# CSB5/XNA_Basecaller

Measured on NVIDIA B200. Metric: signal samples/sec basecalled (sup@v3.3 XNA), higher is better.
Workload: dtype fp16

## Files before the change

### xna_basecaller_b200/csrc/conv3_gemm.cu

```cuda
#include "xb_common.cuh"
#include "xb_ptx.cuh"
#include "xb_gemm.cuh"

using namespace xbptx;

namespace {

constexpr int BM = 128, BN = 192, BK = 64;
constexpr int KBLK = XB_CONV3_K / BK;
constexpr int GROUPS = XB_FEATURES / BN;
constexpr int A_BYTES = BM * BK * 2, B_KB_BYTES = BN * BK * 2;
constexpr int STAGES = 4;
constexpr int STG_BYTES = 32 * 128;
constexpr int OFF_A = KBLK * B_KB_BYTES;
constexpr int OFF_STG = OFF_A + STAGES * A_BYTES;
constexpr int OFF_BIAS = OFF_STG + 8 * STG_BYTES;
constexpr int OFF_BAR = OFF_BIAS + BN * 4;
constexpr int SMEM_BYTES = OFF_BAR + 256 + 1024 ;
constexpr int THREADS = 384;
static_assert(XB_CONV3_K % BK == 0 && XB_FEATURES % BN == 0, "tile plan");
static_assert(OFF_A % 1024 == 0 && OFF_STG % 1024 == 0 && SMEM_BYTES <= 232448, "shared memory plan");

struct Conv3Params {
    int M, T, NB;
    const float *bias;
    const void *col;
    uint16_t *out;
};

__device__ __forceinline__ float tanh_approx(float x) {
    float y;
    asm("tanh.approx.f32 %0, %1;" : "=f"(y) : "f"(x));
    return y;
}
__device__ __forceinline__ void tma_store_3d(const CUtensorMap *m, uint32_t src_smem, int c0, int c1, int c2) {
    asm volatile("cp.async.bulk.tensor.3d.global.shared::cta.bulk_group [%0, {%2, %3, %4}], [%1];"
                 ::"l"(m), "r"(src_smem), "r"(c0), "r"(c1), "r"(c2) : "memory");
}
__device__ __forceinline__ void bulk_wait_group_read0() { asm volatile("cp.async.bulk.wait_group.read 0;" ::: "memory"); }

__global__ void __launch_bounds__(THREADS, 1)
conv3_kernel(const __grid_constant__ CUtensorMap tmA, const __grid_constant__ CUtensorMap tmB,
             const __grid_constant__ CUtensorMap tmO, const Conv3Params p) {
    extern __shared__ uint8_t smem_raw[];
    uint8_t *smem = reinterpret_cast<uint8_t *>((reinterpret_cast<uintptr_t>(smem_raw) + 1023) & ~uintptr_t(1023));
    float *sbias = reinterpret_cast<float *>(smem + OFF_BIAS);
    uint64_t *full = reinterpret_cast<uint64_t *>(smem + OFF_BAR);
    uint64_t *empty = full + STAGES;
    uint64_t *acc_full = empty + STAGES;
    uint64_t *acc_empty = acc_full + 2;
    uint64_t *w_full = acc_empty + 2;
    uint32_t *tmem_holder = reinterpret_cast<uint32_t *>(w_full + 1);

    const int warp = threadIdx.x >> 5, lane = threadIdx.x & 31;
    const int group = blockIdx.x % GROUPS, worker = blockIdx.x / GROUPS, workers = gridDim.x / GROUPS;
    const int n0 = group * BN;
    const int ntiles = (p.M + BM - 1) / BM;

    if (warp == 0 && lane == 0) {
        prefetch_tmap(&tmA);
        prefetch_tmap(&tmB);
        prefetch_tmap(&tmO);
        for (int s = 0; s < STAGES; s++) {
            mbar_init(&full[s], 1);
            mbar_init(&empty[s], 1);
        }
        for (int b = 0; b < 2; b++) {
            mbar_init(&acc_full[b], 1);
            mbar_init(&acc_empty[b], 4);
        }
        mbar_init(w_full, 1);
        fence_barrier_init();
    }
    if (warp == 2) {
        tmem_alloc(tmem_holder, 512);
        tmem_relinquish();
    }
    for (int i = threadIdx.x; i < BN; i += THREADS) sbias[i] = p.bias[n0 + i];
    tc_fence_before();
    __syncthreads();
    tc_fence_after();
    const uint32_t tmem_base = *tmem_holder;

    if (warp == 0) {
        if (elect_one()) {
            mbar_expect_tx(w_full, KBLK * B_KB_BYTES);
            for (int kb = 0; kb < KBLK; kb++) tma_load_2d(smem + kb * B_KB_BYTES, &tmB, w_full, kb * BK, n0);
            uint32_t it = 0;
            for (int tile = worker; tile < ntiles; tile += workers) {
                const int ahead = tile + 2 * workers;
                if (group == 0 && ahead < ntiles) {
                    const int rows = min(BM, p.M - ahead * BM);
                    const char *src = reinterpret_cast<const char *>(p.col) + (size_t)ahead * BM * (XB_CONV3_K * 2);
                    const uint32_t bytes = (uint32_t)rows * (XB_CONV3_K * 2);
                    for (uint32_t off = 0; off < bytes; off += 16384) prefetch_l2_bulk(src + off, min(16384u, bytes - off));
                }
                for (int kb = 0; kb < KBLK; kb++, it++) {
                    const int s = it % STAGES;
                    mbar_wait(&empty[s], ((it / STAGES) & 1) ^ 1);
                    mbar_expect_tx(&full[s], A_BYTES);
                    tma_load_2d(smem + OFF_A + s * A_BYTES, &tmA, &full[s], kb * BK, tile * BM);
                }
            }
        }
    } else if (warp == 1) {
        constexpr uint32_t idesc = umma_idesc_f16(0u, BM, BN);
        mbar_wait(w_full, 0);
        uint32_t it = 0, ti = 0;
        for (int tile = worker; tile < ntiles; tile += workers, ti++) {
            const int buf = ti & 1;
            mbar_wait(&acc_empty[buf], ((ti >> 1) & 1) ^ 1);
            tc_fence_after();
            const uint32_t d = tmem_base + buf * BN;
            for (int kb = 0; kb < KBLK; kb++, it++) {
                const int s = it % STAGES;
                mbar_wait(&full[s], (it / STAGES) & 1);
                tc_fence_after();
                if (elect_one()) {
                    const uint32_t a_addr = smem_u32(smem + OFF_A + s * A_BYTES);
                    const uint32_t b_addr = smem_u32(smem + kb * B_KB_BYTES);
#pragma unroll
                    for (int k = 0; k < BK / 16; k++)
                        mma_f16_ss(d, umma_desc_sw128(a_addr + k * 32), umma_desc_sw128(b_addr + k * 32), idesc, (kb | k) != 0);
                    mma_commit(&empty[s]);
                    if (kb == KBLK - 1) mma_commit(&acc_full[buf]);
                }
                __syncwarp();
            }
        }
    } else if (warp >= 4) {
        const int set = (warp - 4) >> 2, q = warp & 3;
        const uint32_t lane_base = tmem_base + ((uint32_t)(q * 32) << 16);
        const uint32_t stg = smem_u32(smem + OFF_STG + (set * 4 + q) * STG_BYTES);
        const uint32_t row_s = stg + lane * 128;
        uint32_t ti = 0;
        for (int tile = worker; tile < ntiles; tile += workers, ti++) {
            if ((int)(ti & 1) != set) continue;
            const int buf = ti & 1;
            mbar_wait(&acc_full[buf], (ti >> 1) & 1);
            tc_fence_after();
            const int m_w = tile * BM + q * 32;
            const int b_w = m_w / p.T, t_w = m_w - b_w * p.T;
#pragma unroll 1
            for (int cb = 0; cb < BN; cb += 64) {
                uint32_t a0[32], a1[32];
                tmem_ld_32x32b_x32(lane_base + buf * BN + cb, a0);
                tmem_ld_32x32b_x32(lane_base + buf * BN + cb + 32, a1);
                tmem_ld_wait();
                if (cb + 64 == BN) {
                    tc_fence_before();
                    __syncwarp();
                    if (lane == 0) mbar_arrive(&acc_empty[buf]);
                }
                const float *bs = sbias + cb;
                uint32_t pk[32];
#pragma unroll
                for (int e = 0; e < 32; e++) {
                    const int c = 2 * e;
                    float v0 = __uint_as_float(c < 32 ? a0[c & 31] : a1[c & 31]) + bs[c];
                    float v1 = __uint_as_float(c < 32 ? a0[(c + 1) & 31] : a1[(c + 1) & 31]) + bs[c + 1];
                    v0 = v0 * fmaf(tanh_approx(0.5f * v0), 0.5f, 0.5f);
                    v1 = v1 * fmaf(tanh_approx(0.5f * v1), 0.5f, 0.5f);
                    pk[e] = xb16<false>::pack(v0, v1);
                }
                if (lane == 0) bulk_wait_group_read0();
                __syncwarp();
#pragma unroll
                for (int j = 0; j < 8; j++)
                    sts_v4(row_s + (uint32_t)((j ^ (lane & 7)) << 4), make_uint4(pk[4 * j], pk[4 * j + 1], pk[4 * j + 2], pk[4 * j + 3]));
                if (t_w + 32 <= p.T) {
                    fence_proxy_async();
                    __syncwarp();
                    if (lane == 0) {
                        if (b_w < p.NB) tma_store_3d(&tmO, stg, n0 + cb, t_w, b_w);
                        bulk_commit_group();
                    }
                } else {
                    __syncwarp();
                    const int m = m_w + lane;
                    if (m < p.M) {
                        const int b = m / p.T, t = m - b * p.T;
                        uint16_t *o = p.out + ((size_t)t * p.NB + b) * XB_FEATURES + n0 + cb;
#pragma unroll
                        for (int j = 0; j < 8; j++)
                            reinterpret_cast<uint4 *>(o)[j] = lds_v4(row_s + (uint32_t)((j ^ (lane & 7)) << 4));
                    }
                    __syncwarp();
                }
            }
        }
        if (lane == 0) bulk_wait_group0();
        tc_fence_before();
    }
    __syncthreads();
    if (warp == 2) {
        tc_fence_after();
        tmem_dealloc(tmem_base, 512);
    }
}

}

int xb_conv3_launch(xb_handle *h, const void *col, const void *w3, const float *bias, void *out_tnc, int T, int N, cudaStream_t s) {
    const uint64_t M = (uint64_t)N * T;
    CUtensorMap tmA, tmB, tmO;
    if (int rc = xb_make_tmap_2d(h, &tmA, col, M, XB_CONV3_K, XB_CONV3_K)) return rc;
    if (int rc = xb_make_tmap_2d_box(h, &tmB, w3, XB_FEATURES, XB_CONV3_K, XB_CONV3_K, BK, BN, 1)) return rc;
    {
        const uint64_t dims[3] = {XB_FEATURES, (uint64_t)T, (uint64_t)N};
        const uint64_t st[2] = {(uint64_t)N * XB_FEATURES * 2, XB_FEATURES * 2};
        const uint32_t box[3] = {64, 32, 1};
        if (int rc = xb_make_tmap_nd(h, &tmO, out_tnc, 3, 2, dims, st, box)) return rc;
    }
    static bool configured[64] = {};
    if (!configured[h->device & 63]) {
        XB_CUDA(h, cudaFuncSetAttribute(conv3_kernel, cudaFuncAttributeMaxDynamicSharedMemorySize, SMEM_BYTES));
        configured[h->device & 63] = true;
    }
    Conv3Params p;
    p.M = (int)M; p.T = T; p.NB = N; p.bias = bias; p.col = col; p.out = reinterpret_cast<uint16_t *>(out_tnc);
    const int ntiles = (int)((M + BM - 1) / BM);
    int workers = (h->num_sms > 0 ? h->num_sms : 148) / GROUPS;
    if (workers > ntiles) workers = ntiles;
    conv3_kernel<<<GROUPS * workers, THREADS, SMEM_BYTES, s>>>(tmA, tmB, tmO, p);
    XB_LAUNCH_CHECK(h);
    return XB_OK;
}
```

### xna_basecaller_b200/csrc/conv_stem.cu

```cuda
#include "xb_common.cuh"

namespace {

constexpr int TT = 32;
constexpr int NP2 = 5 * TT + 14;
constexpr int NP1 = NP2 + 4;
constexpr int NPX = NP1 + 4;
constexpr int THREADS = 256;

__device__ __forceinline__ float swishf(float x) { return x * __fdividef(1.0f, 1.0f + __expf(-x)); }

template <typename SIG> __device__ __forceinline__ float load_sig(const SIG *p, size_t i);
template <> __device__ __forceinline__ float load_sig<float>(const float *p, size_t i) { return __ldg(p + i); }
template <> __device__ __forceinline__ float load_sig<__half>(const __half *p, size_t i) { return __half2float(p[i]); }
template <> __device__ __forceinline__ float load_sig<int16_t>(const int16_t *p, size_t i) { return (float)p[i]; }

template <bool BF16, typename SIG>
__global__ void __launch_bounds__(THREADS)
conv12_im2col_kernel(const SIG *__restrict__ signal, int L, int T, const float *__restrict__ w1,
                     const float *__restrict__ b1, const float *__restrict__ w2, const float *__restrict__ b2,
                     uint16_t *__restrict__ rows) {
    using X = xb16<BF16>;
    __shared__ float sx[NPX];
    __shared__ float s1[NP1][4];
    __shared__ __align__(16) uint16_t s2[NP2 + 1][16];
    __shared__ float sw1[20], sb1[4], sw2[320], sb2[16];

    const int b = blockIdx.y, t0 = blockIdx.x * TT, tid = threadIdx.x;
    const int p2_0 = 5 * t0 - 9;
    const int p1_0 = p2_0 - 2, px_0 = p1_0 - 2;
    const SIG *sig = signal + (size_t)b * L;

    for (int i = tid; i < 20; i += THREADS) sw1[i] = w1[i];
    for (int i = tid; i < 4; i += THREADS) sb1[i] = b1[i];
    for (int i = tid; i < 320; i += THREADS) sw2[i] = w2[i];
    for (int i = tid; i < 16; i += THREADS) sb2[i] = b2[i];
    for (int i = tid; i < NPX; i += THREADS) {
        int p = px_0 + i;
        sx[i] = (p >= 0 && p < L) ? load_sig<SIG>(sig, p) : 0.0f;
    }
    __syncthreads();
    for (int i = tid; i < NP1 * 4; i += THREADS) {
        int pos = i >> 2, ch = i & 3, p = p1_0 + pos;
        float v = 0.0f;
        if (p >= 0 && p < L) {
            v = sb1[ch];
#pragma unroll
            for (int k = 0; k < 5; k++) v = fmaf(sw1[ch * 5 + k], sx[pos + k], v);
            v = swishf(v);
        }
        s1[pos][ch] = v;
    }
    __syncthreads();
    for (int i = tid; i < (NP2 + 1) * 16; i += THREADS) {
        int pos = i >> 4, ch = i & 15, p = p2_0 + pos;
        float v = 0.0f;
        if (pos < NP2 && p >= 0 && p < L) {
            v = sb2[ch];
#pragma unroll
            for (int ci = 0; ci < 4; ci++)
#pragma unroll
                for (int k = 0; k < 5; k++) v = fmaf(sw2[(ch * 4 + ci) * 5 + k], s1[pos + k][ci], v);
            v = swishf(v);
        }
        typename X::T hv = X::from(v);
        s2[pos][ch] = *reinterpret_cast<uint16_t *>(&hv);
    }
    __syncthreads();
    const uint4 *s2v = reinterpret_cast<const uint4 *>(&s2[0][0]);
    for (int i = tid; i < TT * 40; i += THREADS) {
        int r = i / 40, v = i - r * 40, t = t0 + r;
        if (t >= T) continue;
        uint4 val = make_uint4(0, 0, 0, 0);
        if (v < 38) val = s2v[r * 10 + v];
        reinterpret_cast<uint4 *>(rows + ((size_t)b * T + t) * XB_CONV3_K)[v] = val;
    }
}

template <bool BF16, typename SIG>
int launch(xb_handle *h, const void *signal, int N, int L, cudaStream_t s) {
    const int T = L / XB_STRIDE;
    dim3 grid((T + TT - 1) / TT, N);
    conv12_im2col_kernel<BF16, SIG><<<grid, THREADS, 0, s>>>(reinterpret_cast<const SIG *>(signal), L, T, h->conv1_w,
                                                             h->conv1_b, h->conv2_w, h->conv2_b,
                                                             reinterpret_cast<uint16_t *>(h->c2));
    XB_LAUNCH_CHECK(h);
    return XB_OK;
}

}

int xb_conv12_im2col(xb_handle *h, const void *signal, int sig_dtype, int N, int L, cudaStream_t s) {
    switch (sig_dtype) {
        case XB_SIG_F32: return launch<false, float>(h, signal, N, L, s);
        case XB_SIG_F16: return launch<false, __half>(h, signal, N, L, s);
        case XB_SIG_I16: return launch<false, int16_t>(h, signal, N, L, s);
    }
    return xb_fail(h, XB_ERR_ARG, "unknown signal dtype %d", sig_dtype);
}
```

### xna_basecaller_b200/csrc/xb_api.cu

```cuda
#include <stdarg.h>
#include <stdlib.h>
#include <string.h>

#include "xb_common.cuh"
#include "xb_gemm.cuh"

thread_local std::string xb_global_err;

int xb_fail(xb_handle *h, int code, const char *fmt, ...) {
    char buf[512];
    va_list ap;
    va_start(ap, fmt);
    vsnprintf(buf, sizeof buf, fmt, ap);
    va_end(ap);
    if (h) h->err = buf;
    xb_global_err = buf;
    return code;
}

int xb_conv12_im2col(xb_handle *h, const void *signal, int sig_dtype, int N, int L, cudaStream_t s);
int xb_lstm_recurrence_persistent(xb_handle *h, int layer, void *y_tnc, int T, int N, int reverse, cudaStream_t s, void *save = nullptr);
int xb_inproj_launch(xb_handle *h, const void *x, const void *w_ih, const float *bias, void *gates, int M, cudaStream_t s);
int xb_head_astationary_launch(xb_handle *h, const void *x, const void *w, int w_rows, const float *bias, int head_rows,
                               float *scores, int ldo, int M, int exp_out, cudaStream_t s);
int xb_preprocess_impl(xb_handle *h, const int16_t *raw, const int64_t *read_offset, const int32_t *read_len,
                       const double *scaling, const int32_t *offset, int n_reads, float *out, int32_t *out_len,
                       float *stats, cudaStream_t s);
int xb_ctc_loss_bwd_impl(xb_handle *h, const float *scores, int T, int N, const int32_t *targets, int Lmax,
                         const int32_t *lengths, int normalise, const float *grad_loss, float *alpha_ws, float *grad,
                         cudaStream_t s);
int xb_ctc_loss_impl(xb_handle *h, const float *scores, int T, int N, const int32_t *targets, int Lmax,
                     const int32_t *lengths, int normalise, float *loss, cudaStream_t s);
int xb_stitch_impl(xb_handle *h, const int8_t *rows, int T, const int32_t *chunk_first, const int32_t *chunk_count,
                   const int32_t *read_len, int n_reads, int chunksize, int overlap, int stride, int reverse, int8_t *out,
                   int out_stride, int32_t *out_len, cudaStream_t s);

void xb_train_free(xb_handle *h);
int xb_beam_search_impl(xb_handle *h, const float *scores, const float *beta, int T, int N, int beam_width, float beam_cut,
                        int8_t *seq, int8_t *qstring, int8_t *moves, int32_t *lens, cudaStream_t s);
int xb_onehot_edges(xb_handle *h, const int32_t *edges_nt, int T, int N, int S, float *post, cudaStream_t s);
int xb_gather_chunks_impl(xb_handle *h, const void *signal, int sig_dtype, const int64_t *read_offset,
                          const int32_t *read_len, const int32_t *chunk_read, const int32_t *chunk_start, int n_chunks,
                          int L, float *out, cudaStream_t s);

namespace {

int ipow(int b, int e) { int r = 1; while (e-- > 0) r *= b; return r; }

template <typename T> int dev_alloc(xb_handle *h, T **p, size_t count) {
    void *q = nullptr;
    cudaError_t e = cudaMalloc(&q, count * sizeof(T));
    if (e != cudaSuccess)
        return xb_fail(h, XB_ERR_NOMEM, "cudaMalloc of %zu bytes failed: %s", count * sizeof(T), cudaGetErrorString(e));
    *p = reinterpret_cast<T *>(q);
    return XB_OK;
}
int dev_alloc_bytes(xb_handle *h, void **p, size_t bytes) { return dev_alloc<uint8_t>(h, reinterpret_cast<uint8_t **>(p), bytes); }

template <bool BF16>
__global__ void repack_kernel(const float *__restrict__ src, uint16_t *__restrict__ dst, int rows_dst, int cols_dst,
                              int rows_src, int cols_src, int mode) {
    size_t i = (size_t)blockIdx.x * blockDim.x + threadIdx.x;
    if (i >= (size_t)rows_dst * cols_dst) return;
    int r = (int)(i / cols_dst), c = (int)(i % cols_dst);
    float v = 0.0f;
    if (mode == 0) {
        if (r < rows_src && c < cols_src) v = src[(size_t)r * cols_src + c];
    } else if (mode == 1) {
        int j = r >> 7, g = (r >> 5) & 3, u = r & 31;
        v = src[(size_t)(g * XB_FEATURES + j * 32 + u) * cols_src + c];
    } else if (mode == 3) {
        int j = r >> 7, u = (r >> 2) & 31, g = r & 3;
        v = src[(size_t)(g * XB_FEATURES + j * 32 + u) * cols_src + c];
    } else if (mode == 4) {
        int j = r >> 7, q = (r >> 5) & 3, g = (r >> 3) & 3, ul = r & 7;
        v = src[(size_t)(g * XB_FEATURES + j * 32 + q * 8 + ul) * cols_src + c];
    } else if (mode == 5 || mode == 6) {
        if (mode == 5) { if (r < cols_src && c < rows_src) v = src[(size_t)c * cols_src + r]; }
        else {
            int tap = r >> 4, ch = r & 15;
            if (tap < XB_WINLEN) v = src[((size_t)c * XB_C2_CH + ch) * XB_WINLEN + tap];
        }
        __nv_bfloat16 bv = __float2bfloat16_rn(v);
        dst[i] = *reinterpret_cast<uint16_t *>(&bv);
        return;
    } else {
        int tap = c >> 4, ch = c & 15;
        if (tap < XB_WINLEN) v = src[((size_t)r * XB_C2_CH + ch) * XB_WINLEN + tap];
    }
    if (BF16) v = __bfloat162float(__float2bfloat16_rn(v));
    __half hv = __float2half_rn(v);
    dst[i] = *reinterpret_cast<uint16_t *>(&hv);
}
__global__ void lstm_bias_kernel(const float *__restrict__ b_ih, const float *__restrict__ b_hh, float *__restrict__ dst,
                                 int mode) {
    int r = blockIdx.x * blockDim.x + threadIdx.x;
    if (r >= XB_GATES) return;
    int j = r >> 7, g = (r >> 5) & 3, u = r & 31;
    if (mode == 3) { u = (r >> 2) & 31; g = r & 3; }
    int s = g * XB_FEATURES + j * 32 + u;
    dst[r] = b_ih[s] + b_hh[s];
}

// ... 14 lines not shown
    XB_REQUIRE(h, T > 0 && N > 0, "T and N must be positive (got T=%d N=%d)", T, N);
    XB_REQUIRE(h, T <= h->max_T && N <= h->max_N, "T=%d N=%d exceed the handle capacity max_T=%d max_N=%d", T, N, h->max_T,
               h->max_N);
    return XB_OK;
}

}

extern "C" {

int xb_abi_version(void) { return XB_ABI_VERSION; }

const char *xb_last_error(const xb_handle *h) { return h ? h->err.c_str() : xb_global_err.c_str(); }

int64_t xb_launch_count(const xb_handle *h) { return h ? h->launches : 0; }

int xb_set_profiling(xb_handle *h, int on) {
    if (!h) return xb_fail(nullptr, XB_ERR_ARG, "NULL handle");
    h->profiling = on != 0;
    return XB_OK;
}

int xb_stage_times(xb_handle *h, float *ms, int *spans) {
    if (!h) return xb_fail(nullptr, XB_ERR_ARG, "NULL handle");
    XB_REQUIRE(h, ms && spans, "NULL buffer");
    for (int i = 0; i < XB_ST_COUNT; i++) { ms[i] = 0.f; spans[i] = 0; }
    for (auto &sp : h->spans) {
        XB_CUDA(h, cudaEventSynchronize(sp.b));
        float t = 0.f;
        XB_CUDA(h, cudaEventElapsedTime(&t, sp.a, sp.b));
        ms[sp.stage] += t;
        spans[sp.stage]++;
        h->event_pool.push_back(sp.a);
        h->event_pool.push_back(sp.b);
    }
    h->spans.clear();
    return XB_OK;
}

int xb_create(xb_handle **out, int device, int max_N, int max_T, int n_base, int state_len, const char *alphabet, int flags) {
    if (!out) return xb_fail(nullptr, XB_ERR_ARG, "xb_create: out is NULL");
    *out = nullptr;
    if (max_N <= 0 || max_T <= 0) return xb_fail(nullptr, XB_ERR_ARG, "xb_create: max_N and max_T must be positive");
    if (!alphabet || (int)strlen(alphabet) != n_base + 1 || n_base + 1 > 15)
        return xb_fail(nullptr, XB_ERR_ARG, "xb_create: alphabet must have n_base+1 letters (blank first)");
    int key = n_base * 10 + state_len;
    if (!(key == 43 || key == 53 || key == 63 || key == 44 || key == 22))
        return xb_fail(nullptr, XB_ERR_UNSUPPORTED, "xb_create: no kernels for n_base=%d state_len=%d", n_base, state_len);
    int ndev = 0;
    cudaError_t e = cudaGetDeviceCount(&ndev);
    if (e != cudaSuccess || ndev == 0)
        return xb_fail(nullptr, XB_ERR_CUDA, "xb_create: no CUDA device (%s); this library has no CPU path",
                       cudaGetErrorString(e));
    if (device < 0 || device >= ndev) return xb_fail(nullptr, XB_ERR_ARG, "xb_create: device %d out of range", device);
    cudaDeviceProp prop;
    if (cudaGetDeviceProperties(&prop, device) != cudaSuccess || prop.major != 10)
        return xb_fail(nullptr, XB_ERR_UNSUPPORTED, "xb_create: device %d is not compute capability 10.x (sm_100a only)", device);
    if (cudaSetDevice(device) != cudaSuccess) return xb_fail(nullptr, XB_ERR_CUDA, "cudaSetDevice(%d) failed", device);

    xb_handle *h = new xb_handle();
    h->device = device;
    h->max_N = max_N;
    h->max_T = max_T;
    h->n_base = n_base;
    h->state_len = state_len;
    h->C = ipow(n_base, state_len);
    h->NZ = n_base + 1;
    h->flags = flags;
    h->bf16 = (flags & XB_FLAG_BF16) != 0;
    h->num_sms = prop.multiProcessorCount;
    strncpy(h->alphabet, alphabet, sizeof h->alphabet - 1);

    const size_t TN = (size_t)max_T * max_N, S = (size_t)h->C * h->NZ;
    int rc = XB_OK;
#define TRY(x) if (rc == XB_OK) rc = (x)
    const size_t VP = (size_t)((h->C + 31) / 32) * 32 + 4;
    TRY(dev_alloc(h, &h->alpha, (TN + max_N) * VP));
    TRY(dev_alloc(h, &h->bmax, (TN + max_N) * VP));
    TRY(dev_alloc(h, &h->lp, (TN + max_N) * VP));
    TRY(dev_alloc(h, &h->logz, (size_t)max_N));
    TRY(dev_alloc(h, &h->seq_dev, TN));
    TRY(dev_alloc(h, &h->lens_dev, (size_t)max_N));
    if (!(flags & XB_FLAG_NO_ENCODER)) {
        TRY(dev_alloc_bytes(h, &h->c2, TN * XB_CONV3_K * 2));
        TRY(dev_alloc_bytes(h, &h->act0, TN * XB_FEATURES * 2));
        TRY(dev_alloc_bytes(h, &h->act1, TN * XB_FEATURES * 2));
        TRY(dev_alloc_bytes(h, &h->gates, TN * XB_GATES * 2));
        TRY(dev_alloc(h, &h->cstate, (size_t)max_N * XB_FEATURES));
        TRY(dev_alloc(h, &h->scores, TN * S));
        TRY(dev_alloc_bytes(h, &h->signal_dev, TN * XB_STRIDE * sizeof(float)));
    }
#undef TRY
    if (rc != XB_OK) {
        xb_global_err = h->err;
        xb_destroy(h);
        return rc;
    }
    *out = h;
    return XB_OK;
}

int xb_destroy(xb_handle *h) {
    if (!h) return XB_OK;
    cudaSetDevice(h->device);
    void *ptrs[] = {h->conv1_w, h->conv1_b, h->conv2_w, h->conv2_b, h->conv3_w, h->conv3_b, h->head_w, h->head_b, h->c2,
                    h->act0, h->act1, h->gates, h->cstate, h->hzero, h->scores, h->signal_dev, h->seq_dev, h->lens_dev,
                    h->alpha, h->bmax, h->lp, h->logz, h->ctc_ws, h->lstm_counters};
    for (void *p : ptrs)
        if (p) cudaFree(p);
    for (void *p : {(void *)h->signal_dev2, (void *)h->seq_dev2, (void *)h->lens_dev2})
        if (p) cudaFree(p);
    if (h->h2d_stream) cudaStreamDestroy(h->h2d_stream);
    if (h->d2h_stream) cudaStreamDestroy(h->d2h_stream);
    for (int i = 0; i < 2; i++)
        for (cudaEvent_t e : {h->ev_h2d[i], h->ev_enc[i], h->ev_dec[i], h->ev_done[i]})
            if (e) cudaEventDestroy(e);
    for (auto &sp : h->spans) { cudaEventDestroy(sp.a); cudaEventDestroy(sp.b); }
    for (auto e : h->event_pool) cudaEventDestroy(e);
    for (auto &l : h->lstm) {
        for (void *p : {l.w_ih, l.w_hh, (void *)l.bias, l.w_ihT, l.w_hhT})
            if (p) cudaFree(p);
    }
    if (h->head_wT) cudaFree(h->head_wT);
    if (h->conv3_wT) cudaFree(h->conv3_wT);
    xb_train_free(h);
    delete h;
    return XB_OK;
}

static int alloc_weights(xb_handle *h) {
    if (h->conv1_w) return XB_OK;
    const int F = XB_FEATURES;
    h->head_rows = ipow(h->n_base, h->state_len + 1);
    h->head_rows_padded = ((h->head_rows + 127) / 128) * 128;
    int rc = XB_OK;
#define TRY(x) if (rc == XB_OK) rc = (x)
    TRY(dev_alloc(h, &h->conv1_w, 20));
    TRY(dev_alloc(h, &h->conv1_b, 4));
    TRY(dev_alloc(h, &h->conv2_w, 320));
    TRY(dev_alloc(h, &h->conv2_b, 16));
    TRY(dev_alloc_bytes(h, &h->conv3_w, (size_t)F * XB_CONV3_K * 2));
    TRY(dev_alloc(h, &h->conv3_b, (size_t)F));
    for (auto &l : h->lstm) {
        TRY(dev_alloc_bytes(h, &l.w_ih, (size_t)XB_GATES * F * 2));
        TRY(dev_alloc_bytes(h, &l.w_hh, (size_t)XB_GATES * F * 2));
        TRY(dev_alloc(h, &l.bias, (size_t)XB_GATES));
    }
    TRY(dev_alloc_bytes(h, &h->head_w, (size_t)h->head_rows_padded * F * 2));
    TRY(dev_alloc(h, &h->head_b, (size_t)h->head_rows_padded));
#undef TRY
    return rc;
}

#define XB_WEIGHTS_PROLOGUE()                                                                          \
    if (!h) return xb_fail(nullptr, XB_ERR_ARG, "NULL handle");                                        \
    XB_REQUIRE(h, !(h->flags & XB_FLAG_NO_ENCODER), "handle was created with XB_FLAG_NO_ENCODER");     \
    cudaStream_t s = reinterpret_cast<cudaStream_t>(stream);                                           \
    XB_CUDA(h, cudaSetDevice(h->device));                                                              \
    if (int rc_ = alloc_weights(h)) return rc_

int xb_load_conv_weights(xb_handle *h, const float *w1, const float *b1, const float *w2, const float *b2,
                         const float *w3, const float *b3, void *stream) {
    XB_WEIGHTS_PROLOGUE();
    XB_REQUIRE(h, w1 && b1 && w2 && b2 && w3 && b3, "NULL convolution weight");
    const int F = XB_FEATURES;
    XB_CUDA(h, cudaMemcpyAsync(h->conv1_w, w1, 20 * 4, cudaMemcpyDeviceToDevice, s));
    XB_CUDA(h, cudaMemcpyAsync(h->conv1_b, b1, 4 * 4, cudaMemcpyDeviceToDevice, s));
    XB_CUDA(h, cudaMemcpyAsync(h->conv2_w, w2, 320 * 4, cudaMemcpyDeviceToDevice, s));
    XB_CUDA(h, cudaMemcpyAsync(h->conv2_b, b2, 16 * 4, cudaMemcpyDeviceToDevice, s));
    if (int rc = repack(h, w3, h->conv3_w, F, XB_CONV3_K, F, XB_C2_CH * XB_WINLEN, 2, s)) return rc;
    if (h->flags & XB_FLAG_TRAIN) {
        if (!h->conv3_wT) { if (int rc = dev_alloc_bytes(h, &h->conv3_wT, (size_t)XB_CONV3_K * F * 2)) return rc; }
        if (int rc = repack(h, w3, h->conv3_wT, XB_CONV3_K, F, F, XB_C2_CH * XB_WINLEN, 6, s)) return rc;
    }
    XB_CUDA(h, cudaMemcpyAsync(h->conv3_b, b3, F * 4, cudaMemcpyDeviceToDevice, s));
    h->loaded |= 1;
    return XB_OK;
}

int xb_load_lstm_weights(xb_handle *h, int layer, const float *w_ih, const float *w_hh, const float *b_ih,
                         const float *b_hh, void *stream) {
    XB_WEIGHTS_PROLOGUE();
    XB_REQUIRE(h, layer >= 0 && layer < 5, "LSTM layer %d out of range", layer);
    XB_REQUIRE(h, w_ih && w_hh && b_ih && b_hh, "NULL LSTM weight");
    const int F = XB_FEATURES;
#ifdef XB_EXPERIMENTS
#define XB_FLAG_LSTM_STEPWISE 4
    const int ih_mode = (h->flags & XB_FLAG_LSTM_STEPWISE) ? 1 : 3;
#else
    const int ih_mode = 3;
#endif
    if (int rc = repack(h, w_ih, h->lstm[layer].w_ih, XB_GATES, F, XB_GATES, F, ih_mode, s)) return rc;
    if (int rc = repack(h, w_hh, h->lstm[layer].w_hh, XB_GATES, F, XB_GATES, F, ih_mode == 3 ? 4 : 1, s)) return rc;
    if (h->flags & XB_FLAG_TRAIN) {
        xb_lstm_weights &lw = h->lstm[layer];
        if (!lw.w_ihT) { if (int rc = dev_alloc_bytes(h, &lw.w_ihT, (size_t)XB_GATES * F * 2)) return rc; }
        if (!lw.w_hhT) { if (int rc = dev_alloc_bytes(h, &lw.w_hhT, (size_t)XB_GATES * F * 2)) return rc; }
        if (int rc = repack(h, w_ih, lw.w_ihT, F, XB_GATES, XB_GATES, F, 5, s)) return rc;
        if (int rc = repack(h, w_hh, lw.w_hhT, F, XB_GATES, XB_GATES, F, 5, s)) return rc;
    }
    lstm_bias_kernel<<<(XB_GATES + 255) / 256, 256, 0, s>>>(b_ih, b_hh, h->lstm[layer].bias, ih_mode);
    XB_LAUNCH_CHECK(h);
    h->loaded |= 2 << layer;
    return XB_OK;
}

int xb_load_head_weights(xb_handle *h, const float *w, const float *b, float scale, float blank_score,
                         int expand_blanks, void *stream) {
    XB_WEIGHTS_PROLOGUE();
    XB_REQUIRE(h, w != nullptr, "NULL head weight");
    const int F = XB_FEATURES;
    if (int rc = repack(h, w, h->head_w, h->head_rows_padded, F, h->head_rows, F, 0, s)) return rc;
    if (h->flags & XB_FLAG_TRAIN) {
        if (!h->head_wT) { if (int rc = dev_alloc_bytes(h, &h->head_wT, (size_t)h->head_rows_padded * F * 2)) return rc; }
        if (int rc = repack(h, w, h->head_wT, F, h->head_rows_padded, h->head_rows, F, 5, s)) return rc;
    }
    XB_CUDA(h, cudaMemsetAsync(h->head_b, 0, (size_t)h->head_rows_padded * 4, s));
    if (b) XB_CUDA(h, cudaMemcpyAsync(h->head_b, b, (size_t)h->head_rows * 4, cudaMemcpyDeviceToDevice, s));
    h->scale = scale;
    h->blank_score = blank_score;
    h->expand_blanks = expand_blanks;
    h->loaded |= 64;
    return XB_OK;
}

int xb_load_weights(xb_handle *h, const float *const *w, int n_tensors, float scale, float blank_score, int expand_blanks,
                    void *stream) {
    if (!h) return xb_fail(nullptr, XB_ERR_ARG, "xb_load_weights: NULL handle");
    XB_REQUIRE(h, w && n_tensors == XB_NUM_WEIGHTS, "expected %d weight tensors, got %d", XB_NUM_WEIGHTS, n_tensors);
    for (int i = 0; i < n_tensors; i++) XB_REQUIRE(h, w[i] != nullptr, "weight tensor %d is NULL", i);
    if (int rc = xb_load_conv_weights(h, w[0], w[1], w[2], w[3], w[4], w[5], stream)) return rc;
    for (int l = 0; l < 5; l++) {
        const float *const *lw = w + 6 + 4 * l;
        if (int rc = xb_load_lstm_weights(h, l, lw[0], lw[1], lw[2], lw[3], stream)) return rc;
    }
    return xb_load_head_weights(h, w[26], w[27], scale, blank_score, expand_blanks, stream);
}

int xb_conv_stem_fwd(xb_handle *h, const void *signal, int sig_dtype, int N, int L, void *out_tnc, void *stream) {
    if (!h) return xb_fail(nullptr, XB_ERR_ARG, "NULL handle");
    if (!(h->loaded & 1)) return xb_fail(h, XB_ERR_STATE, "convolution weights have not been loaded (xb_load_weights)");
    XB_REQUIRE(h, signal && out_tnc, "NULL buffer");
    XB_REQUIRE(h, L > 0 && L % XB_STRIDE == 0, "chunk length %d must be a positive multiple of the stride %d", L, XB_STRIDE);
    const int T = L / XB_STRIDE;
    if (int rc = check_tn(h, T, N)) return rc;
    cudaStream_t s = reinterpret_cast<cudaStream_t>(stream);
    {
        xb_stage_timer tm(h, XB_ST_CONV12, s);
        if (int rc = xb_conv12_im2col(h, signal, sig_dtype, N, L, s)) return rc;
    }
    xb_stage_timer tm(h, XB_ST_CONV3, s);
    return xb_conv3_launch(h, h->c2, h->conv3_w, h->conv3_b, out_tnc, T, N, s);
}

int xb_lstm_fwd(xb_handle *h, int layer, const void *x_tnc, void *y_tnc, int T, int N, int reverse, void *stream) {
    if (!h) return xb_fail(nullptr, XB_ERR_ARG, "NULL handle");
    XB_REQUIRE(h, layer >= 0 && layer < 5, "LSTM layer %d out of range", layer);
    if (!(h->loaded & (2 << layer))) return xb_fail(h, XB_ERR_STATE, "weights of LSTM layer %d have not been loaded", layer);
    XB_REQUIRE(h, x_tnc && y_tnc && x_tnc != y_tnc, "x and y must be distinct non-NULL buffers");
    if (int rc = check_tn(h, T, N)) return rc;
    cudaStream_t s = reinterpret_cast<cudaStream_t>(stream);
    const xb_lstm_weights &lw = h->lstm[layer];
    {
        xb_stage_timer tm(h, XB_ST_INPROJ, s);
#ifdef XB_EXPERIMENTS
        static const bool generic = getenv("XB_INPROJ_GENERIC") != nullptr;
        if (generic) {
            CUtensorMap tmA, tmB;
            if (int rc = xb_make_tmap_2d(h, &tmA, x_tnc, (uint64_t)T * N, XB_FEATURES, XB_FEATURES)) return rc;
            if (int rc = xb_make_tmap_2d(h, &tmB, lw.w_ih, XB_GATES, XB_FEATURES, XB_FEATURES)) return rc;
            GemmParams p;
            p.M = T * N; p.N = XB_GATES; p.K = XB_FEATURES;
            p.bias = lw.bias; p.out = h->gates; p.ldo = XB_GATES;
            if (int rc = xb_gemm_launch(h, EPI_INPROJ, tmA, tmB, p, s)) return rc;
        } else
#endif
        if (int rc = xb_inproj_launch(h, x_tnc, lw.w_ih, lw.bias, h->gates, T * N, s)) return rc;
    }
    xb_stage_timer tm(h, XB_ST_LSTM_REC, s);
#ifdef XB_EXPERIMENTS
    if (h->flags & XB_FLAG_LSTM_STEPWISE) {
        CUtensorMap tmH, tmW;
        if (int rc = xb_make_tmap_2d(h, &tmH, y_tnc, (uint64_t)T * N, XB_FEATURES, XB_FEATURES)) return rc;
        if (int rc = xb_make_tmap_2d(h, &tmW, lw.w_hh, XB_GATES, XB_FEATURES, XB_FEATURES)) return rc;
        for (int i = 0; i < T; i++) {
            const int t = reverse ? T - 1 - i : i;
            const int tp = reverse ? t + 1 : t - 1;
            GemmParams p;
            p.M = N; p.N = XB_GATES; p.K = XB_FEATURES;
            p.a_row_offset = (i == 0) ? 0 : tp * N;
            p.out = y_tnc; p.NB = N;
            p.gates = h->gates; p.cstate = h->cstate;
            p.t_cur = t; p.first = (i == 0);
            if (int rc = xb_gemm_launch(h, EPI_LSTM, tmH, tmW, p, s)) return rc;
        }
        return XB_OK;
    }
#endif
    return xb_lstm_recurrence_persistent(h, layer, y_tnc, T, N, reverse, s);
}

int xb_lstm_stack_fwd(xb_handle *h, void *x_tnc, void *y_tnc, int T, int N, void *stream) {
    if (!h) return xb_fail(nullptr, XB_ERR_ARG, "NULL handle");
    XB_REQUIRE(h, x_tnc && y_tnc && x_tnc != y_tnc, "x and y must be distinct non-NULL buffers");
    void *a = x_tnc, *b = y_tnc;
    for (int l = 0; l < 5; l++) {
        if (int rc = xb_lstm_fwd(h, l, a, b, T, N, (l % 2) == 0, stream)) return rc;
        void *t = a; a = b; b = t;
    }
    return XB_OK;
}

static int head_fwd(xb_handle *h, const void *x_tnc, float *scores, int T, int N, int exp_out, void *stream) {
    if (!h) return xb_fail(nullptr, XB_ERR_ARG, "NULL handle");
    if (!(h->loaded & 64)) return xb_fail(h, XB_ERR_STATE, "CRF head weights have not been loaded (xb_load_weights)");
    XB_REQUIRE(h, x_tnc && scores, "NULL buffer");
    if (int rc = check_tn(h, T, N)) return rc;
    cudaStream_t s = reinterpret_cast<cudaStream_t>(stream);
    xb_stage_timer tm(h, XB_ST_HEAD, s);
#ifdef XB_EXPERIMENTS
    static const bool tile_gemm = getenv("XB_HEAD_GENERIC") != nullptr;
    if (tile_gemm) {
        CUtensorMap tmA, tmB;
        if (int rc = xb_make_tmap_2d(h, &tmA, x_tnc, (uint64_t)T * N, XB_FEATURES, XB_FEATURES)) return rc;
        if (int rc = xb_make_tmap_2d(h, &tmB, h->head_w, h->head_rows_padded, XB_FEATURES, XB_FEATURES)) return rc;
        GemmParams p;
        p.M = T * N; p.N = h->head_rows_padded; p.K = XB_FEATURES;
        p.bias = h->head_b; p.out = scores;
        p.ldo = h->expand_blanks ? h->C * h->NZ : h->head_rows;
        p.n_base = h->n_base; p.head_rows = h->head_rows; p.expand = h->expand_blanks;
        p.scale = h->scale; p.blank = h->blank_score;
        return xb_gemm_launch(h, EPI_HEAD, tmA, tmB, p, s);
// ... 259 lines not shown
```

### xna_basecaller_b200/csrc/xb_common.cuh

```cuda
#pragma once

#include <cuda_runtime.h>
#include <cuda_fp16.h>
#include <cuda_bf16.h>
#include <cuda.h>
#include <stdint.h>
#include <stdio.h>
#include <string>
#include <vector>

#include "../../include/xna_basecaller.h"

#define XB_FEATURES 768
#define XB_GATES (4 * XB_FEATURES)
#define XB_STRIDE 5
#define XB_WINLEN 19
#define XB_C2_CH 16
#define XB_C2_HALO 9
#define XB_CONV3_K 320

struct xb_lstm_weights {
    void *w_ih = nullptr;
    void *w_hh = nullptr;
    float *bias = nullptr;
    void *w_ihT = nullptr;
    void *w_hhT = nullptr;
};

enum { XB_ST_CONV12 = 0, XB_ST_CONV3, XB_ST_INPROJ, XB_ST_LSTM_REC, XB_ST_HEAD, XB_ST_CRF_ALPHA, XB_ST_CRF_BACKWARD,
       XB_ST_CRF_VITERBI, XB_ST_TRAIN_BPTT, XB_ST_TRAIN_TRANSPOSE, XB_ST_TRAIN_WGRAD, XB_ST_TRAIN_XGRAD, XB_ST_TRAIN_HEAD_CONV,
       XB_ST_COUNT };

struct xb_prof_span { int stage; cudaEvent_t a, b; };

struct xb_handle {
    int device = 0;
    bool profiling = false;
    std::vector<xb_prof_span> spans;
    std::vector<cudaEvent_t> event_pool;
    int max_N = 0, max_T = 0;
    int n_base = 0, state_len = 0, C = 0, NZ = 0;
    int flags = 0;
    bool bf16 = false;
    int loaded = 0;
    char alphabet[16] = {0};
    int num_sms = 0;
    int64_t launches = 0;
    std::string err;

    float *conv1_w = nullptr, *conv1_b = nullptr, *conv2_w = nullptr, *conv2_b = nullptr;
    void *conv3_w = nullptr;
    float *conv3_b = nullptr;
    xb_lstm_weights lstm[5];
    void *head_w = nullptr;
    float *head_b = nullptr;
    int head_rows = 0, head_rows_padded = 0;
    float scale = 5.0f, blank_score = 2.0f;
    int expand_blanks = 1;

    void *c2 = nullptr;
    void *act0 = nullptr, *act1 = nullptr;
    void *gates = nullptr;
    float *cstate = nullptr;
    void *hzero = nullptr;
    float *scores = nullptr;
    void *signal_dev = nullptr;
    int8_t *seq_dev = nullptr;
    int32_t *lens_dev = nullptr;
    void *signal_dev2 = nullptr;
    int8_t *seq_dev2 = nullptr;
    int32_t *lens_dev2 = nullptr;
    cudaStream_t h2d_stream = nullptr, d2h_stream = nullptr;
    cudaEvent_t ev_h2d[2] = {nullptr, nullptr}, ev_enc[2] = {nullptr, nullptr}, ev_dec[2] = {nullptr, nullptr},
                ev_done[2] = {nullptr, nullptr};
    bool slot_used[2] = {false, false};

    float *alpha = nullptr;
    float *bmax = nullptr;
    float *lp = nullptr;
    float *logz = nullptr;
    float *ctc_ws = nullptr;
    int *lstm_counters = nullptr;

    void *head_wT = nullptr;
    void *conv3_wT = nullptr;
    struct xb_train_ws *train = nullptr;

    void *encode_tiled = nullptr;
};

extern thread_local std::string xb_global_err;

struct xb_stage_timer {
    xb_handle *h; cudaStream_t s; int idx = -1;
    xb_stage_timer(xb_handle *h_, int stage, cudaStream_t s_) : h(h_), s(s_) {
        if (!h->profiling) return;
        auto get = [&]() { cudaEvent_t e; if (!h->event_pool.empty()) { e = h->event_pool.back(); h->event_pool.pop_back(); }
                           else cudaEventCreate(&e); return e; };
        xb_prof_span sp{stage, get(), get()};
        cudaEventRecord(sp.a, s);
        h->spans.push_back(sp);
        idx = (int)h->spans.size() - 1;
// ... 64 lines not shown
```

### xna_basecaller_b200/csrc/xb_gemm.cuh

```cuda
#pragma once
#include "xb_common.cuh"

enum { EPI_F32 = 0, EPI_CONV3 = 1, EPI_INPROJ = 2, EPI_HEAD = 3, EPI_LSTM = 4, EPI_BF16OUT = 5, EPI_CONV3_BWD = 7 };

struct GemmParams {
    int M = 0, N = 0, K = 0;
    int a_row_offset = 0;
    int split_k = 1;
    const float *bias = nullptr;
    void *out = nullptr;
    int ldo = 0;
    int T = 0, NB = 0;
    int n_base = 0, head_rows = 0, expand = 0;
    float scale = 0.f, blank = 0.f;
    const void *gates = nullptr;
    float *cstate = nullptr;
    int t_cur = 0, first = 0;
    const void *dy = nullptr;
};

int xb_make_tmap_2d(xb_handle *h, CUtensorMap *out, const void *base, uint64_t rows, uint64_t K, uint64_t ld);
int xb_make_tmap_2d_box(xb_handle *h, CUtensorMap *out, const void *base, uint64_t rows, uint64_t K, uint64_t ld,
                        uint32_t box_inner, uint32_t box_rows, int swizzle128);
int xb_make_tmap_hview(xb_handle *h, CUtensorMap *out, const void *base, uint64_t rows, uint32_t box_rows,
                       uint32_t box_kblocks);
int xb_make_tmap_nd(xb_handle *h, CUtensorMap *out, const void *base, int rank, int elem_bytes, const uint64_t *dims,
                    const uint64_t *strides_bytes, const uint32_t *box);

struct BpttMaps {
    CUtensorMap dz_rows;
    CUtensorMap w_hhT;
    CUtensorMap saved;
    CUtensorMap saved_c;
    CUtensorMap dz_out;
};
struct BpttStep {
    int N = 0, t_cur = 0, t_prev = -1, t_next = -1;
    const void *dy = nullptr;
    float *dcstate = nullptr;
};
int xb_bptt_make_maps(xb_handle *h, BpttMaps *m, const void *dz, const void *w_hhT, const void *saved, int T, int N);
int xb_bptt_step_launch(xb_handle *h, const BpttMaps &m, const BpttStep &p, bool dependent, cudaStream_t s);
int xb_conv3_launch(xb_handle *h, const void *col, const void *w3, const float *bias, void *out_tnc, int T, int N, cudaStream_t s);
int xb_gemm_launch(xb_handle *h, int epi, const CUtensorMap &tmA, const CUtensorMap &tmB, const GemmParams &p,
                   cudaStream_t s, bool bf16_operands = false);
```

Measured before the change: 84.64 million.

## Replace explicit conv3 im2col buffer with overlapping strided slab view

The conv1/conv2 stem now writes a compact per-batch slab of conv2 outputs (16 channels per position, padded to T+4 steps) instead of materializing the full 320-wide im2col rows. The conv3 GEMM reads the A operand through a TMA tensor map whose row pitch equals the stride, so successive rows overlap in memory and the im2col is formed implicitly. This removes most of the write and read traffic of the duplicated im2col buffer. In exchange the GEMM computes a few padded rows per batch that the epilogue must mask out, which it does with the new TS row indexing.

```diff
diff --git a/xna_basecaller_b200/csrc/conv3_gemm.cu b/xna_basecaller_b200/csrc/conv3_gemm.cu
--- a/xna_basecaller_b200/csrc/conv3_gemm.cu
+++ b/xna_basecaller_b200/csrc/conv3_gemm.cu
@@ -18,13 +18,14 @@
 constexpr int OFF_BAR = OFF_BIAS + BN * 4;
 constexpr int SMEM_BYTES = OFF_BAR + 256 + 1024 ;
 constexpr int THREADS = 384;
+constexpr int ROW_PITCH = XB_STRIDE * XB_C2_CH * 2, ROW_BYTES = XB_WINLEN * XB_C2_CH * 2;
 static_assert(XB_CONV3_K % BK == 0 && XB_FEATURES % BN == 0, "tile plan");
 static_assert(OFF_A % 1024 == 0 && OFF_STG % 1024 == 0 && SMEM_BYTES <= 232448, "shared memory plan");
 
 struct Conv3Params {
-    int M, T, NB;
+    int M, T, TS, NB;
     const float *bias;
-    const void *col;
+    const void *slab;
     uint16_t *out;
 };
 
@@ -89,10 +90,10 @@
             uint32_t it = 0;
             for (int tile = worker; tile < ntiles; tile += workers) {
                 const int ahead = tile + 2 * workers;
-                if (group == 0 && ahead < ntiles) {
-                    const int rows = min(BM, p.M - ahead * BM);
-                    const char *src = reinterpret_cast<const char *>(p.col) + (size_t)ahead * BM * (XB_CONV3_K * 2);
-                    const uint32_t bytes = (uint32_t)rows * (XB_CONV3_K * 2);
+                if (group == 0 && ahead * BM < p.M - 3) {
+                    const int rows = min(BM, p.M - 3 - ahead * BM);
+                    const char *src = reinterpret_cast<const char *>(p.slab) + (size_t)ahead * BM * ROW_PITCH;
+                    const uint32_t bytes = (uint32_t)(rows - 1) * ROW_PITCH + ROW_BYTES;
                     for (uint32_t off = 0; off < bytes; off += 16384) prefetch_l2_bulk(src + off, min(16384u, bytes - off));
                 }
                 for (int kb = 0; kb < KBLK; kb++, it++) {
@@ -140,7 +141,7 @@
             mbar_wait(&acc_full[buf], (ti >> 1) & 1);
             tc_fence_after();
             const int m_w = tile * BM + q * 32;
-            const int b_w = m_w / p.T, t_w = m_w - b_w * p.T;
+            const int b_w = m_w / p.TS, t_w = m_w - b_w * p.TS;
 #pragma unroll 1
             for (int cb = 0; cb < BN; cb += 64) {
                 uint32_t a0[32], a1[32];
@@ -168,7 +169,7 @@
 #pragma unroll
                 for (int j = 0; j < 8; j++)
                     sts_v4(row_s + (uint32_t)((j ^ (lane & 7)) << 4), make_uint4(pk[4 * j], pk[4 * j + 1], pk[4 * j + 2], pk[4 * j + 3]));
-                if (t_w + 32 <= p.T) {
+                if (t_w + 32 <= p.TS) {
                     fence_proxy_async();
                     __syncwarp();
                     if (lane == 0) {
@@ -178,8 +179,8 @@
                 } else {
                     __syncwarp();
                     const int m = m_w + lane;
-                    if (m < p.M) {
-                        const int b = m / p.T, t = m - b * p.T;
+                    const int b = m / p.TS, t = m - b * p.TS;
+                    if (b < p.NB && t < p.T) {
                         uint16_t *o = p.out + ((size_t)t * p.NB + b) * XB_FEATURES + n0 + cb;
 #pragma unroll
                         for (int j = 0; j < 8; j++)
@@ -201,10 +202,11 @@
 
 }
 
-int xb_conv3_launch(xb_handle *h, const void *col, const void *w3, const float *bias, void *out_tnc, int T, int N, cudaStream_t s) {
-    const uint64_t M = (uint64_t)N * T;
+int xb_conv3_launch(xb_handle *h, const void *slab, const void *w3, const float *bias, void *out_tnc, int T, int N, cudaStream_t s) {
+    const int TS = xb_slab_steps(T);
+    const uint64_t M = (uint64_t)N * TS;
     CUtensorMap tmA, tmB, tmO;
-    if (int rc = xb_make_tmap_2d(h, &tmA, col, M, XB_CONV3_K, XB_CONV3_K)) return rc;
+    if (int rc = xb_make_tmap_2d(h, &tmA, slab, M - 3, ROW_BYTES / 2, ROW_PITCH / 2)) return rc;
     if (int rc = xb_make_tmap_2d_box(h, &tmB, w3, XB_FEATURES, XB_CONV3_K, XB_CONV3_K, BK, BN, 1)) return rc;
     {
         const uint64_t dims[3] = {XB_FEATURES, (uint64_t)T, (uint64_t)N};
@@ -218,7 +220,7 @@
         configured[h->device & 63] = true;
     }
     Conv3Params p;
-    p.M = (int)M; p.T = T; p.NB = N; p.bias = bias; p.col = col; p.out = reinterpret_cast<uint16_t *>(out_tnc);
+    p.M = (int)M; p.T = T; p.TS = TS; p.NB = N; p.bias = bias; p.slab = slab; p.out = reinterpret_cast<uint16_t *>(out_tnc);
     const int ntiles = (int)((M + BM - 1) / BM);
     int workers = (h->num_sms > 0 ? h->num_sms : 148) / GROUPS;
     if (workers > ntiles) workers = ntiles;
diff --git a/xna_basecaller_b200/csrc/conv_stem.cu b/xna_basecaller_b200/csrc/conv_stem.cu
--- a/xna_basecaller_b200/csrc/conv_stem.cu
+++ b/xna_basecaller_b200/csrc/conv_stem.cu
@@ -3,9 +3,7 @@
 namespace {
 
 constexpr int TT = 32;
-constexpr int NP2 = 5 * TT + 14;
-constexpr int NP1 = NP2 + 4;
-constexpr int NPX = NP1 + 4;
+constexpr int SP = 5 * TT;
 constexpr int THREADS = 256;
 
 __device__ __forceinline__ float swishf(float x) { return x * __fdividef(1.0f, 1.0f + __expf(-x)); }
@@ -15,19 +13,22 @@
 template <> __device__ __forceinline__ float load_sig<__half>(const __half *p, size_t i) { return __half2float(p[i]); }
 template <> __device__ __forceinline__ float load_sig<int16_t>(const int16_t *p, size_t i) { return (float)p[i]; }
 
-template <bool BF16, typename SIG>
+template <bool SLAB, typename SIG>
 __global__ void __launch_bounds__(THREADS)
-conv12_im2col_kernel(const SIG *__restrict__ signal, int L, int T, const float *__restrict__ w1,
-                     const float *__restrict__ b1, const float *__restrict__ w2, const float *__restrict__ b2,
-                     uint16_t *__restrict__ rows) {
-    using X = xb16<BF16>;
+conv12_kernel(const SIG *__restrict__ signal, int L, int T, const float *__restrict__ w1, const float *__restrict__ b1,
+              const float *__restrict__ w2, const float *__restrict__ b2, uint16_t *__restrict__ out) {
+    using X = xb16<false>;
+    constexpr int NP2 = SLAB ? SP : 5 * TT + 14, NS2 = SLAB ? NP2 : NP2 + 1;
+    constexpr int NP1 = NP2 + 4, NPX = NP1 + 4;
     __shared__ float sx[NPX];
     __shared__ float s1[NP1][4];
-    __shared__ __align__(16) uint16_t s2[NP2 + 1][16];
+    __shared__ __align__(16) uint16_t s2[NS2][16];
     __shared__ float sw1[20], sb1[4], sw2[320], sb2[16];
 
-    const int b = blockIdx.y, t0 = blockIdx.x * TT, tid = threadIdx.x;
-    const int p2_0 = 5 * t0 - 9;
+    const int b = blockIdx.y, tid = threadIdx.x;
+    const int t0 = blockIdx.x * TT;
+    const int q0 = blockIdx.x * SP;
+    const int p2_0 = (SLAB ? q0 : 5 * t0) - XB_C2_HALO;
     const int p1_0 = p2_0 - 2, px_0 = p1_0 - 2;
     const SIG *sig = signal + (size_t)b * L;
 
@@ -52,7 +53,7 @@
         s1[pos][ch] = v;
     }
     __syncthreads();
-    for (int i = tid; i < (NP2 + 1) * 16; i += THREADS) {
+    for (int i = tid; i < NS2 * 16; i += THREADS) {
         int pos = i >> 4, ch = i & 15, p = p2_0 + pos;
         float v = 0.0f;
         if (pos < NP2 && p >= 0 && p < L) {
@@ -68,33 +69,47 @@
     }
     __syncthreads();
     const uint4 *s2v = reinterpret_cast<const uint4 *>(&s2[0][0]);
-    for (int i = tid; i < TT * 40; i += THREADS) {
-        int r = i / 40, v = i - r * 40, t = t0 + r;
-        if (t >= T) continue;
-        uint4 val = make_uint4(0, 0, 0, 0);
-        if (v < 38) val = s2v[r * 10 + v];
-        reinterpret_cast<uint4 *>(rows + ((size_t)b * T + t) * XB_CONV3_K)[v] = val;
+    if constexpr (SLAB) {
+        const int pitch = XB_STRIDE * xb_slab_steps(T), n = 2 * min(SP, pitch - q0);
+        uint4 *dst = reinterpret_cast<uint4 *>(out + ((size_t)b * pitch + q0) * XB_C2_CH);
+        for (int i = tid; i < n; i += THREADS) dst[i] = s2v[i];
+    } else {
+        for (int i = tid; i < TT * 40; i += THREADS) {
+            int r = i / 40, v = i - r * 40, t = t0 + r;
+            if (t >= T) continue;
+            uint4 val = make_uint4(0, 0, 0, 0);
+            if (v < 38) val = s2v[r * 10 + v];
+            reinterpret_cast<uint4 *>(out + ((size_t)b * T + t) * XB_CONV3_K)[v] = val;
+        }
     }
 }
 
-template <bool BF16, typename SIG>
+template <bool SLAB, typename SIG>
 int launch(xb_handle *h, const void *signal, int N, int L, cudaStream_t s) {
     const int T = L / XB_STRIDE;
-    dim3 grid((T + TT - 1) / TT, N);
-    conv12_im2col_kernel<BF16, SIG><<<grid, THREADS, 0, s>>>(reinterpret_cast<const SIG *>(signal), L, T, h->conv1_w,
-                                                             h->conv1_b, h->conv2_w, h->conv2_b,
-                                                             reinterpret_cast<uint16_t *>(h->c2));
+    dim3 grid(SLAB ? (XB_STRIDE * xb_slab_steps(T) + SP - 1) / SP : (T + TT - 1) / TT, N);
+    conv12_kernel<SLAB, SIG><<<grid, THREADS, 0, s>>>(reinterpret_cast<const SIG *>(signal), L, T, h->conv1_w, h->conv1_b,
+                                                      h->conv2_w, h->conv2_b, reinterpret_cast<uint16_t *>(h->c2));
     XB_LAUNCH_CHECK(h);
     return XB_OK;
 }
 
+template <bool SLAB>
+int launch_dtype(xb_handle *h, const void *signal, int sig_dtype, int N, int L, cudaStream_t s) {
+    switch (sig_dtype) {
+        case XB_SIG_F32: return launch<SLAB, float>(h, signal, N, L, s);
+        case XB_SIG_F16: return launch<SLAB, __half>(h, signal, N, L, s);
+        case XB_SIG_I16: return launch<SLAB, int16_t>(h, signal, N, L, s);
+    }
+    return xb_fail(h, XB_ERR_ARG, "unknown signal dtype %d", sig_dtype);
+}
+
+}
+
+int xb_conv12_slab(xb_handle *h, const void *signal, int sig_dtype, int N, int L, cudaStream_t s) {
+    return launch_dtype<true>(h, signal, sig_dtype, N, L, s);
 }
 
 int xb_conv12_im2col(xb_handle *h, const void *signal, int sig_dtype, int N, int L, cudaStream_t s) {
-    switch (sig_dtype) {
-        case XB_SIG_F32: return launch<false, float>(h, signal, N, L, s);
-        case XB_SIG_F16: return launch<false, __half>(h, signal, N, L, s);
-        case XB_SIG_I16: return launch<false, int16_t>(h, signal, N, L, s);
-    }
-    return xb_fail(h, XB_ERR_ARG, "unknown signal dtype %d", sig_dtype);
+    return launch_dtype<false>(h, signal, sig_dtype, N, L, s);
 }
diff --git a/xna_basecaller_b200/csrc/xb_api.cu b/xna_basecaller_b200/csrc/xb_api.cu
--- a/xna_basecaller_b200/csrc/xb_api.cu
+++ b/xna_basecaller_b200/csrc/xb_api.cu
@@ -1,3 +1,4 @@
+#include <algorithm>
 #include <stdarg.h>
 #include <stdlib.h>
 #include <string.h>
@@ -18,7 +19,7 @@
     return code;
 }
 
-int xb_conv12_im2col(xb_handle *h, const void *signal, int sig_dtype, int N, int L, cudaStream_t s);
+int xb_conv12_slab(xb_handle *h, const void *signal, int sig_dtype, int N, int L, cudaStream_t s);
 int xb_lstm_recurrence_persistent(xb_handle *h, int layer, void *y_tnc, int T, int N, int reverse, cudaStream_t s, void *save = nullptr);
 int xb_inproj_launch(xb_handle *h, const void *x, const void *w_ih, const float *bias, void *gates, int M, cudaStream_t s);
 int xb_head_astationary_launch(xb_handle *h, const void *x, const void *w, int w_rows, const float *bias, int head_rows,
@@ -199,7 +200,8 @@
     TRY(dev_alloc(h, &h->seq_dev, TN));
     TRY(dev_alloc(h, &h->lens_dev, (size_t)max_N));
     if (!(flags & XB_FLAG_NO_ENCODER)) {
-        TRY(dev_alloc_bytes(h, &h->c2, TN * XB_CONV3_K * 2));
+        const size_t slab = (size_t)max_N * xb_slab_steps(max_T) * XB_STRIDE * XB_C2_CH * 2;
+        TRY(dev_alloc_bytes(h, &h->c2, (flags & XB_FLAG_TRAIN) ? std::max(slab, TN * XB_CONV3_K * 2) : slab));
         TRY(dev_alloc_bytes(h, &h->act0, TN * XB_FEATURES * 2));
         TRY(dev_alloc_bytes(h, &h->act1, TN * XB_FEATURES * 2));
         TRY(dev_alloc_bytes(h, &h->gates, TN * XB_GATES * 2));
@@ -364,7 +366,7 @@
     cudaStream_t s = reinterpret_cast<cudaStream_t>(stream);
     {
         xb_stage_timer tm(h, XB_ST_CONV12, s);
-        if (int rc = xb_conv12_im2col(h, signal, sig_dtype, N, L, s)) return rc;
+        if (int rc = xb_conv12_slab(h, signal, sig_dtype, N, L, s)) return rc;
     }
     xb_stage_timer tm(h, XB_ST_CONV3, s);
     return xb_conv3_launch(h, h->c2, h->conv3_w, h->conv3_b, out_tnc, T, N, s);
diff --git a/xna_basecaller_b200/csrc/xb_common.cuh b/xna_basecaller_b200/csrc/xb_common.cuh
--- a/xna_basecaller_b200/csrc/xb_common.cuh
+++ b/xna_basecaller_b200/csrc/xb_common.cuh
@@ -18,6 +18,8 @@
 #define XB_C2_CH 16
 #define XB_C2_HALO 9
 #define XB_CONV3_K 320
+
+__host__ __device__ inline int xb_slab_steps(int T) { return T + 4; }
 
 struct xb_lstm_weights {
     void *w_ih = nullptr;
diff --git a/xna_basecaller_b200/csrc/xb_gemm.cuh b/xna_basecaller_b200/csrc/xb_gemm.cuh
--- a/xna_basecaller_b200/csrc/xb_gemm.cuh
+++ b/xna_basecaller_b200/csrc/xb_gemm.cuh
@@ -41,6 +41,6 @@
 };
 int xb_bptt_make_maps(xb_handle *h, BpttMaps *m, const void *dz, const void *w_hhT, const void *saved, int T, int N);
 int xb_bptt_step_launch(xb_handle *h, const BpttMaps &m, const BpttStep &p, bool dependent, cudaStream_t s);
-int xb_conv3_launch(xb_handle *h, const void *col, const void *w3, const float *bias, void *out_tnc, int T, int N, cudaStream_t s);
+int xb_conv3_launch(xb_handle *h, const void *slab, const void *w3, const float *bias, void *out_tnc, int T, int N, cudaStream_t s);
 int xb_gemm_launch(xb_handle *h, int epi, const CUtensorMap &tmA, const CUtensorMap &tmB, const GemmParams &p,
                    cudaStream_t s, bool bf16_operands = false);
```

Result: no change. 84.71 million, median of 6 (+0.1%).
